# SamuelCancilla2/radar-point-cloud-tracking

Hardware: AMD Instinct MI355X
Metric: Mpoints/s clustered+tracked, 1024-echo synthetic frames; 1/2/4/8-GPU scaling (higher is better)
Workload: dtype u8 echo / f32 geometry / f64 distance

## Files before the change

### radar-point-cloud-tracking_amd/csrc/k1_emit.h

```cpp
#pragma once
#include <cstdint>

#if defined(__HIPCC__) || defined(__CUDACC__)
#define RPT_K1_HD __host__ __device__ __forceinline__
#else
#define RPT_K1_HD inline
#endif

namespace rpt {

constexpr int kStageSlots = 512;

struct EmitStride {
  uint32_t stride;
  uint32_t shift;
  bool pow2;
};
RPT_K1_HD EmitStride emit_stride(uint32_t stride) {
  return EmitStride{stride, (uint32_t)__builtin_ctz(stride), (stride & (stride - 1u)) == 0u};
}

struct EmitSpan {
  uint32_t first;
  uint32_t m;
  uint32_t rank0;
};

RPT_K1_HD uint32_t emit_ceil(uint32_t a, const EmitStride& es, uint32_t* rem) {
  const uint32_t q = es.pow2 ? (a >> es.shift) : a / es.stride;
  const uint32_t r = es.pow2 ? (a & (es.stride - 1u)) : a - q * es.stride;
  if (rem) *rem = r;
  return q + (r != 0u ? 1u : 0u);
}

RPT_K1_HD EmitSpan emit_span(uint32_t rank, uint32_t total, const EmitStride& es) {
  uint32_t rem;
  EmitSpan s;
  s.first = emit_ceil(rank, es, &rem);
  s.m = emit_ceil(rank + total, es, nullptr) - s.first;
  s.rank0 = rem != 0u ? es.stride - rem : 0u;
  return s;
}

RPT_K1_HD bool emit_staged(const EmitSpan& s) { return s.m != 0u && s.m <= (uint32_t)kStageSlots; }

}
```

### radar-point-cloud-tracking_amd/csrc/polar.hip

```cpp
#include <algorithm>
#include <cmath>
#include <cstdlib>

#include "common.h"
#include "k1_emit.h"

#pragma clang fp contract(off)

namespace rpt {
namespace {

constexpr int kBlock = 256;
constexpr int kWavesPerBlock = kBlock / kWave;

template <class T>
__device__ __forceinline__ float to_f(T v) {
  return (float)v;
}

template <class T>
struct Vec;
template <>
struct Vec<uint8_t> {
  static constexpr int N = 16;
// ... 275 lines not shown
    b.v[1] = max(b.v[1], part[4 * i + 1]);
    b.v[2] = min(b.v[2], part[4 * i + 2]);
    b.v[3] = max(b.v[3], part[4 * i + 3]);
  }
  __shared__ uint32_t sm[4 * kWavesPerBlock];
  b.store_block(out - 4 * blockIdx.x, sm, 1);
}

__device__ __forceinline__ void group_to_lds(GroupLds& L, int lane, const uint32_t (&m)[kGroupRows],
                                             const int (&incl)[kGroupRows],
                                             const uint4 (&vv)[kGroupRows]) {
#pragma unroll
  for (int k = 0; k < kGroupRows; ++k) {
    L.incl[k][lane] = (uint16_t)incl[k];
    L.mask[k][lane] = (uint16_t)m[k];
    *reinterpret_cast<uint4*>(&L.bytes[k][lane * 4]) = vv[k];
  }
  wave_lds_sync();
}

__device__ __forceinline__ uint32_t kept_entry(const GroupLds& L,
                                               const uint32_t (&rb)[kGroupRows + 1], uint32_t i) {
  const int k = (i >= rb[1]) + (i >= rb[2]) + (i >= rb[3]);
  const int ir = (int)(i - rb[k]);
  const uint16_t* inc = L.incl[k];
  int lo = 0;
#pragma unroll
  for (int step = 32; step > 0; step >>= 1)
    if (inc[lo + step - 1] <= ir) lo += step;
  const uint32_t msk = L.mask[k][lo];
  const int j = ir - ((int)inc[lo] - __popc(msk));
  const int bit = nth_bit16(msk, (uint32_t)j);
  const int bin = lo * 16 + bit;
  const uint32_t w = L.bytes[k][bin >> 2];
  return ((uint32_t)k << 18) | ((uint32_t)bin << 8) | __builtin_amdgcn_ubfe(w, 8u * (bin & 3), 8u);
}

__device__ __forceinline__ uint32_t phase_base(uint32_t ph, uint32_t total) {
  uint32_t b = 0u;
#pragma unroll
  for (uint32_t j = 0u; j < 3u; ++j) b += (j < ph) ? ((total + 3u - j) >> 2) : 0u;
  return b;
}
__device__ __forceinline__ uint32_t stage_pos(uint32_t i, uint32_t total, bool ph4) {
  return ph4 ? phase_base(i & 3u, total) + (i >> 2) : i;
}
struct StageBases {
  uint32_t b1, b2, b3;
  __device__ explicit StageBases(uint32_t total)
      : b1((total + 3u) >> 2), b2(b1 + ((total + 2u) >> 2)), b3(b2 + ((total + 1u) >> 2)) {}
  __device__ uint32_t pos(uint32_t i) const {
    const uint32_t r = i & 3u;
    return (r == 0u ? 0u : (r == 1u ? b1 : (r == 2u ? b2 : b3))) + (i >> 2);
  }
};

template <bool HI, bool STAGE>
__global__ __launch_bounds__(kBlock) void k_group_count_u8(const uint8_t* __restrict__ echo,
                                                          uint32_t n_groups, GroupMap gm,
                                                          uint32_t K,
                                                          int32_t* __restrict__ group_count,
                                                          uint32_t* __restrict__ entries,
                                                          int ph4) {
  const int lane = threadIdx.x & 63;
  const uint32_t wave0 = __builtin_amdgcn_readfirstlane(blockIdx.x * kWavesPerBlock +
                                                        threadIdx.x / 64);
  const uint32_t n_waves = gridDim.x * kWavesPerBlock;
  const uint32_t dq = n_waves / gm.gpf, dr = n_waves - dq * gm.gpf;
  uint32_t gf = wave0 / gm.gpf, gr = wave0 - gf * gm.gpf;
  for (uint32_t g0 = wave0; g0 < n_groups; g0 += n_waves) {
    const uint32_t grp = g0;
    const uint32_t f = gf;
    const int r0 = (int)gr * kGroupRows;
    const int64_t row0 = (int64_t)f * gm.rows + r0;
    const int nr = min(kGroupRows, gm.rows - r0);
    gf += dq;
    gr += dr;
    if (gr >= gm.gpf) {
      gr -= gm.gpf;
      ++gf;
    }
    uint4 v[kGroupRows];
#pragma unroll
    for (int k = 0; k < kGroupRows; ++k) {
      const u32x4 q = (k < nr) ? __builtin_nontemporal_load(reinterpret_cast<const u32x4*>(
                                     echo + (row0 + k) * 1024 + lane * 16))
                               : u32x4{0u, 0u, 0u, 0u};
      v[k] = make_uint4(q.x, q.y, q.z, q.w);
    }
    if constexpr (STAGE) {
      uint32_t m[kGroupRows];
      int incl[kGroupRows];
#pragma unroll
      for (int k = 0; k < kGroupRows; ++k)
        m[k] = (k < nr) ? mask16(keep_bits<HI>(v[k].x, K), keep_bits<HI>(v[k].y, K),
                                 keep_bits<HI>(v[k].z, K), keep_bits<HI>(v[k].w, K))
                        : 0u;
      static_assert(kGroupRows == 4, "rows are scanned in pairs");
      uint32_t rb[kGroupRows + 1];
      rb[0] = 0;
#pragma unroll
      for (int k = 0; k < kGroupRows; k += 2) {
        const int pair = wave_incl_scan_dpp(__popc(m[k]) | (__popc(m[k + 1]) << 16));
        incl[k] = pair & 0xffff;
        incl[k + 1] = (int)((uint32_t)pair >> 16);
        const uint32_t tot = (uint32_t)__builtin_amdgcn_readlane(pair, 63);
        rb[k + 1] = rb[k] + (tot & 0xffffu);
        rb[k + 2] = rb[k + 1] + (tot >> 16);
      }
      const uint32_t total = rb[kGroupRows];
      if (total != 0u && total <= (uint32_t)kStageSlots) {
        uint32_t* e = entries + (int64_t)grp * kStageSlots;
        __shared__ GroupLds s_lds[kWavesPerBlock];
        GroupLds& L = s_lds[threadIdx.x / 64];
        group_to_lds(L, lane, m, incl, v);
        const StageBases sb(total);
        for (uint32_t i = (uint32_t)lane; i < total; i += 64u)
          e[ph4 ? sb.pos(i) : i] = kept_entry(L, rb, i);
        wave_lds_sync();
      }
      if (lane == 0) group_count[grp] = (int32_t)total;
      continue;
    } else {
      uint32_t c = 0;
#pragma unroll
      for (int k = 0; k < kGroupRows; ++k) {
        if (k >= nr) break;
        c += __popc(keep_bits<HI>(v[k].x, K)) + __popc(keep_bits<HI>(v[k].y, K)) +
             __popc(keep_bits<HI>(v[k].z, K)) + __popc(keep_bits<HI>(v[k].w, K));
      }
      int s = (int)c;
#pragma unroll
      for (int off = 32; off > 0; off >>= 1) s += __shfl_xor(s, off);
      if (lane == 0) group_count[grp] = s;
    }
  }
}

template <int W>
struct CountTotals {
  uint32_t t[2][W];
};
template <bool HI, int W>
__global__ __launch_bounds__(64 * W) void k_group_count_u8_files(
    const uint8_t* __restrict__ echo, GroupMap gm, uint32_t K, EmitStride es,
    int32_t* __restrict__ group_count, uint32_t* __restrict__ entries) {
  __shared__ GroupLds s_lds[W];
  __shared__ CountTotals<W> s_tot;
  const int lane = threadIdx.x & 63;
  const uint32_t w = __builtin_amdgcn_readfirstlane(threadIdx.x / 64);
  const uint32_t f = blockIdx.x;
  const int64_t file_row0 = (int64_t)f * gm.rows;
  const uint32_t n_rounds = (gm.gpf + W - 1) / W;
  auto load_group = [&](uint32_t gi, u32x4 (&q)[kGroupRows]) -> int {
    const int r0 = (int)gi * kGroupRows;
    const int nr = gi < gm.gpf ? min(kGroupRows, gm.rows - r0) : 0;
#pragma unroll
    for (int k = 0; k < kGroupRows; ++k)
      q[k] = (k < nr) ? __builtin_nontemporal_load(reinterpret_cast<const u32x4*>(
                            echo + (file_row0 + r0 + k) * 1024 + lane * 16))
                      : u32x4{0u, 0u, 0u, 0u};
    return nr;
  };
  u32x4 nx[kGroupRows];
  int nr_next = load_group(w, nx);
  uint32_t rank = 0u;
  for (uint32_t r = 0u; r < n_rounds; ++r) {
    const uint32_t gi = r * W + w;
    const int nr = nr_next;
    uint4 v[kGroupRows];
#pragma unroll
    for (int k = 0; k < kGroupRows; ++k) v[k] = make_uint4(nx[k].x, nx[k].y, nx[k].z, nx[k].w);
    nr_next = load_group(gi + W, nx);
    uint32_t m[kGroupRows];
    int incl[kGroupRows];
#pragma unroll
    for (int k = 0; k < kGroupRows; ++k)
      m[k] = (k < nr) ? mask16(keep_bits<HI>(v[k].x, K), keep_bits<HI>(v[k].y, K),
                               keep_bits<HI>(v[k].z, K), keep_bits<HI>(v[k].w, K))
                      : 0u;
    static_assert(kGroupRows == 4, "rows are scanned in pairs");
    uint32_t rb[kGroupRows + 1];
    rb[0] = 0;
#pragma unroll
    for (int k = 0; k < kGroupRows; k += 2) {
      const int pair = wave_incl_scan_dpp(__popc(m[k]) | (__popc(m[k + 1]) << 16));
      incl[k] = pair & 0xffff;
      incl[k + 1] = (int)((uint32_t)pair >> 16);
      const uint32_t tot = (uint32_t)__builtin_amdgcn_readlane(pair, 63);
      rb[k + 1] = rb[k] + (tot & 0xffffu);
      rb[k + 2] = rb[k + 1] + (tot >> 16);
    }
    const uint32_t total = rb[kGroupRows];
    uint32_t my_rank = rank;
    if constexpr (W > 1) {
      const uint32_t par = r & 1u;
      if (lane == 0) s_tot.t[par][w] = total;
      __syncthreads();
      uint32_t below = 0u, all = 0u;
      static_assert(W <= 4, "the wave totals are summed as scalars");
#pragma unroll
      for (uint32_t j = 0u; j < (uint32_t)W; ++j) {
        const uint32_t t = __builtin_amdgcn_readfirstlane(s_tot.t[par][j]);
        below += j < w ? t : 0u;
        all += t;
      }
      my_rank += below;
      rank += all;
    } else {
      rank += total;
    }
    if (nr == 0) continue;
    const EmitSpan sp = emit_span(my_rank, total, es);
    const int64_t grp = (int64_t)f * gm.gpf + gi;
    if (emit_staged(sp)) {
      uint32_t* e = entries + grp * kStageSlots;
      GroupLds& L = s_lds[w];
      group_to_lds(L, lane, m, incl, v);
      for (uint32_t j = (uint32_t)lane; j < sp.m; j += 64u)
        e[j] = kept_entry(L, rb, sp.rank0 + j * es.stride);
      wave_lds_sync();
    }
    if (lane == 0) group_count[grp] = (int32_t)total;
  }
}

constexpr int64_t kCus = 256;
constexpr int64_t kEmittedMinFiles = 1500;
inline int64_t busiest_cu_files(int64_t n_files) { return (n_files + kCus - 1) / kCus; }
inline bool staged_emitted(int64_t n_files) {
  return n_files >= kEmittedMinFiles && n_files * 20 >= busiest_cu_files(n_files) * kCus * 19;
}

inline int count_waves_per_file(int64_t n_files) {
  const int64_t per_cu = busiest_cu_files(n_files);
  return per_cu <= 7 ? 4 : (per_cu <= 15 ? 2 : 1);
}

__global__ void k_file_counts_groups(const int64_t* __restrict__ gprefix, int64_t n_files,
                                     uint32_t gpf, int stride, int64_t* __restrict__ file_out) {
  for (int64_t f = (int64_t)blockIdx.x * blockDim.x + threadIdx.x; f < n_files;
       f += (int64_t)gridDim.x * blockDim.x) {
    const int64_t kept = gprefix[(f + 1) * gpf] - gprefix[f * gpf];
    file_out[f] = (kept + stride - 1) / stride;
  }
}

template <bool HI, bool STAGED, bool LIST = false, class VT = float>
__global__ __launch_bounds__(kBlock, 8) void k_group_write_u8(
    const uint8_t* __restrict__ echo, uint32_t n_groups, GroupMap gm, uint32_t K, int stride,
    const float* __restrict__ scale, const float* __restrict__ cos_t,
    const float* __restrict__ sin_t, const int32_t* __restrict__ gain,
    const int64_t* __restrict__ gprefix, const int64_t* __restrict__ file_offsets,
    int files_per_frame, float* __restrict__ x, float* __restrict__ y, VT* __restrict__ val,
    int32_t* __restrict__ gain_out, int32_t* __restrict__ pf_out, int64_t cap,
    const uint32_t* __restrict__ entries, bool emitted,
    const uint32_t* __restrict__ list = nullptr, const uint32_t* __restrict__ list_n = nullptr,
    uint32_t* __restrict__ bpart = nullptr) {
  __shared__ GroupLds s_lds[kWavesPerBlock];
  XyBounds xb;
  const int lane = threadIdx.x & 63;
  GroupLds& L = s_lds[threadIdx.x / 64];
  const uint32_t wave0 = blockIdx.x * kWavesPerBlock + threadIdx.x / 64;
  const uint32_t n_waves = gridDim.x * kWavesPerBlock;
  const uint32_t us = (uint32_t)stride;
  const EmitStride es = emit_stride(us);
  const float inv_bins = 1.0f / 1024.0f;
  const uint32_t n_items = LIST ? *list_n : n_groups;
  for (uint32_t g0 = wave0; g0 < n_items; g0 += n_waves) {
    const uint32_t grp = __builtin_amdgcn_readfirstlane(LIST ? list[g0] : g0);
    uint32_t f;
    int64_t row0;
    int nr;
    group_rows(gm, grp, &f, &row0, &nr);
    float g_sc = 0.f, g_c = 0.f, g_s = 0.f;
    if (lane < nr) {
      g_sc = scale[row0 + lane];
      g_c = cos_t[row0 + lane];
      g_s = sin_t[row0 + lane];
    }
    float r_sc[kGroupRows], r_c[kGroupRows], r_s[kGroupRows];
#pragma unroll
    for (int k = 0; k < kGroupRows; ++k) {
      r_sc[k] = __builtin_bit_cast(float, __builtin_amdgcn_readlane(__builtin_bit_cast(int, g_sc), k));
      r_c[k] = __builtin_bit_cast(float, __builtin_amdgcn_readlane(__builtin_bit_cast(int, g_c), k));
      r_s[k] = __builtin_bit_cast(float, __builtin_amdgcn_readlane(__builtin_bit_cast(int, g_s), k));
    }
    const int64_t gp0 = gprefix[grp];
    const uint32_t rank = (uint32_t)(gp0 - gprefix[(int64_t)f * gm.gpf]);
    const uint32_t total = (uint32_t)(gprefix[grp + 1] - gp0);
    const EmitSpan sp = emit_span(rank, total, es);
    if (sp.m == 0u) continue;
    const uint32_t first = sp.first, last = sp.first + sp.m;
    const int64_t out0 = file_offsets[f];
    const int32_t g = gain ? gain[f] : 0;
    const int32_t fr = (int32_t)(f / (uint32_t)files_per_frame);
    const bool staged =
        STAGED && (emitted ? emit_staged(sp) : total <= (uint32_t)kStageSlots);
    uint32_t rb[kGroupRows + 1];
    if (!staged) {
      uint4 vv[kGroupRows];
#pragma unroll
      for (int k = 0; k < kGroupRows; ++k)
        vv[k] = (k < nr) ? *reinterpret_cast<const uint4*>(echo + (row0 + k) * 1024 + lane * 16)
                         : make_uint4(0u, 0u, 0u, 0u);
      uint32_t m[kGroupRows];
      int incl[kGroupRows];
#pragma unroll
      for (int k = 0; k < kGroupRows; ++k) {
        m[k] = (k < nr) ? mask16(keep_bits<HI>(vv[k].x, K), keep_bits<HI>(vv[k].y, K),
                                 keep_bits<HI>(vv[k].z, K), keep_bits<HI>(vv[k].w, K))
                        : 0u;
        incl[k] = wave_incl_scan_dpp(__popc(m[k]));
      }
      rb[0] = 0;
#pragma unroll
      for (int k = 0; k < kGroupRows; ++k)
        rb[k + 1] = rb[k] + (uint32_t)__builtin_amdgcn_readlane(incl[k], 63);
      group_to_lds(L, lane, m, incl, vv);
    }
    const uint32_t* e = entries + (int64_t)grp * kStageSlots;
    for (uint32_t o = first + (uint32_t)lane; o < last; o += 64u) {
      const int64_t oo = out0 + o;
      if (oo >= cap) break;
      const uint32_t i = sp.rank0 + (o - first) * us;
      const uint32_t ent = !staged  ? kept_entry(L, rb, i)
                           : emitted ? e[o - first]
                                     : e[stage_pos(i, total, us == 4u)];
      const int rk = (int)(ent >> 18);
      const float sc = rk == 0 ? r_sc[0] : (rk == 1 ? r_sc[1] : (rk == 2 ? r_sc[2] : r_sc[3]));
      const float cc = rk == 0 ? r_c[0] : (rk == 1 ? r_c[1] : (rk == 2 ? r_c[2] : r_c[3]));
      const float ss = rk == 0 ? r_s[0] : (rk == 1 ? r_s[1] : (rk == 2 ? r_s[2] : r_s[3]));
      const float rr = sc * inv_bins * (float)((ent >> 8) & 1023u);
      const float px = rr * cc, py = rr * ss;
      x[oo] = px;
      y[oo] = py;
      if (bpart) xb.add(px, py);
      val[oo] = (VT)(ent & 0xffu);
      if (gain_out) gain_out[oo] = g;
      if (pf_out) pf_out[oo] = fr;
    }
    if (!staged) wave_lds_sync();
  }
  if (bpart)
    xb.store_block(bpart, reinterpret_cast<uint32_t*>(&s_lds[0]),
                   (int)(sizeof(GroupLds) / sizeof(uint32_t) / 4));
}

constexpr int kGsBits = 40;
constexpr uint64_t kGsMask = (1ull << kGsBits) - 1ull;
constexpr uint64_t kUnstaged = 1ull << 63;
constexpr int kTileOut = 1024;
constexpr int kOutPerThread = kTileOut / kBlock;
static_assert(kOutPerThread % 4 == 0, "k_expand_write stores a thread's outputs as 16-B vectors");
constexpr int kWin = 1024;

__global__ __launch_bounds__(kBlock) void k_group_starts(const int64_t* __restrict__ gprefix,
                                                        const int64_t* __restrict__ file_offsets,
                                                        uint32_t n_groups, uint32_t gpf,
                                                        uint32_t stride, bool emitted,
                                                        uint64_t* __restrict__ gword,
                                                        uint32_t* __restrict__ list,
                                                        uint32_t* __restrict__ list_n) {
  constexpr uint32_t kCap = 2048;
  __shared__ uint32_t s_list[kCap];
  __shared__ uint32_t s_n, s_base;
  if (threadIdx.x == 0) s_n = 0u;
  __syncthreads();
  const EmitStride es = emit_stride(stride);
  for (uint32_t b0 = blockIdx.x * kBlock; b0 < n_groups; b0 += gridDim.x * kBlock) {
    const uint32_t g = b0 + threadIdx.x;
    if (g < n_groups) {
      const uint32_t f = g / gpf;
      const int64_t p0 = gprefix[g];
      const uint32_t rank = (uint32_t)(p0 - gprefix[(int64_t)f * gpf]);
      const uint32_t total = (uint32_t)(gprefix[g + 1] - p0);
      const EmitSpan sp = emit_span(rank, total, es);
      const uint64_t gs = (uint64_t)file_offsets[f] + sp.first;
      const uint64_t phase = emitted       ? 0ull
                             : stride == 4u ? (uint64_t)phase_base(sp.rank0, total)
                                            : (uint64_t)sp.rank0;
      const bool un =
          sp.m != 0u && !(emitted ? emit_staged(sp) : total <= (uint32_t)kStageSlots);
      gword[g] = gs | (phase << kGsBits) | (un ? kUnstaged : 0ull);
      if (un) {
        const uint32_t slot = atomicAdd(&s_n, 1u);
        if (slot < kCap)
          s_list[slot] = g;
        else
          list[atomicAdd(list_n, 1u)] = g;
      }
    }
  }
  __syncthreads();
  const uint32_t m = min(s_n, kCap);
  if (threadIdx.x == 0 && m) s_base = atomicAdd(list_n, m);
  __syncthreads();
  for (uint32_t i = threadIdx.x; i < m; i += kBlock) list[s_base + i] = s_list[i];
}

__device__ uint32_t wave_find_group(const uint64_t* __restrict__ gword, uint32_t lo, uint32_t hi,
                                    uint64_t O) {
  const uint32_t lane = threadIdx.x & 63u;
  while (hi - lo > 1u) {
    const uint32_t step = (hi - lo + 63u) / 64u;
    const uint32_t idx = lo + lane * step;
    const bool le = idx < hi && (gword[idx] & kGsMask) <= O;
    const uint64_t m = __ballot(le);
    const uint32_t top = 63u - (uint32_t)__clzll((long long)m);
    lo = __builtin_amdgcn_readfirstlane(lo + top * step);
    hi = min(hi, lo + step);
  }
  return lo;
}

__device__ uint32_t thread_find_group(const uint64_t* __restrict__ gword, uint32_t lo,
                                      uint32_t hi, uint64_t O) {
  while (hi - lo > 1u) {
    const uint32_t mid = lo + (hi - lo) / 2u;
    if ((gword[mid] & kGsMask) <= O)
      lo = mid;
    else
      hi = mid;
  }
  return lo;
}

__device__ __forceinline__ uint32_t lds_find(const uint64_t* s_win, uint32_t wn, uint64_t O) {
  uint32_t lo = 0u;
#pragma unroll
  for (uint32_t step = kWin / 2; step > 0u; step >>= 1)
    if (lo + step < wn && (s_win[lo + step] & kGsMask) <= O) lo += step;
  return lo;
}

template <bool VEC, class VT = float>
__global__ __launch_bounds__(kBlock) void k_expand_write(
    const uint64_t* __restrict__ gword, uint32_t n_groups, GroupMap gm, uint32_t estep,
    const float* __restrict__ scale, const float* __restrict__ cos_t,
    const float* __restrict__ sin_t, const int32_t* __restrict__ gain,
    const int64_t* __restrict__ total_out, int files_per_frame, float* __restrict__ x,
    float* __restrict__ y, VT* __restrict__ val, int32_t* __restrict__ gain_out,
    int32_t* __restrict__ pf_out, int64_t cap, const uint32_t* __restrict__ entries,
    uint32_t* __restrict__ bpart = nullptr) {
  __shared__ uint64_t s_win[kWin];
  __shared__ uint32_t s_glo;
  const int64_t total = min(*total_out, cap);
  const int64_t n_tiles = (total + kTileOut - 1) / kTileOut;
  const int64_t t0 = n_tiles * blockIdx.x / gridDim.x;
  const int64_t t1 = n_tiles * (blockIdx.x + 1) / gridDim.x;
  if (t0 >= t1) {
    if (bpart && threadIdx.x < 4)
      bpart[4 * blockIdx.x + threadIdx.x] = (threadIdx.x & 1) ? 0u : 0xffffffffu;
    return;
  }
  if (threadIdx.x < 64) {
    const uint32_t g = wave_find_group(gword, 0u, n_groups, (uint64_t)t0 * kTileOut);
    if (threadIdx.x == 0) s_glo = g;
  }
  __syncthreads();
  constexpr int kWinPer = kWin / kBlock;
  uint64_t wv[kWinPer];
  auto load_win = [&](uint32_t glo_) {
    const uint32_t wn_ = min((uint32_t)kWin, n_groups - glo_);
#pragma unroll
    for (int q = 0; q < kWinPer; ++q) {
      const uint32_t j = threadIdx.x + q * kBlock;
      wv[q] = j < wn_ ? gword[glo_ + j] : ~0ull;
    }
  };
  auto store_win = [&]() {
#pragma unroll
    for (int q = 0; q < kWinPer; ++q) s_win[threadIdx.x + q * kBlock] = wv[q];
  };
  uint32_t glo = s_glo;
  XyBounds xb;
  load_win(glo);
  store_win();
  __syncthreads();
  const float inv_bins = 1.0f / 1024.0f;
  for (int64_t t = t0; t < t1; ++t) {
    const uint32_t wn = min((uint32_t)kWin, n_groups - glo);
    const bool truncated = glo + wn < n_groups;
    const uint64_t O0 = (uint64_t)t * kTileOut;
    auto word = [&](uint32_t g) -> uint64_t {
      return (g - glo < wn) ? s_win[g - glo] : gword[g];
    };
    auto next_gs = [&](uint32_t g) -> uint64_t {
      return g + 1u < n_groups ? (word(g + 1u) & kGsMask) : ~0ull;
    };
    const uint64_t Ob = O0 + (uint64_t)threadIdx.x * kOutPerThread;
    uint32_t grp[kOutPerThread], idx[kOutPerThread];
    bool ok[kOutPerThread];
    if ((int64_t)Ob < total) {
      const uint32_t j = lds_find(s_win, wn, Ob);
      uint32_t g = (j == wn - 1u && truncated) ? thread_find_group(gword, glo + j, n_groups, Ob)
                                               : glo + j;
      uint64_t w = word(g), nx = next_gs(g);
#pragma unroll
      for (int k = 0; k < kOutPerThread; ++k) {
        const uint64_t O = Ob + k;
        const bool in = (int64_t)O < total;
        while (in && O >= nx) {
          ++g;
          w = word(g);
          nx = next_gs(g);
        }
        ok[k] = in && !(w & kUnstaged);
        grp[k] = g;
        const uint32_t d = (uint32_t)O - (uint32_t)w;
        idx[k] = d * estep + (uint32_t)((w & ~kUnstaged) >> kGsBits);
      }
    } else {
#pragma unroll
      for (int k = 0; k < kOutPerThread; ++k) {
        ok[k] = false;
        grp[k] = glo;
        idx[k] = 0u;
      }
    }
    if (threadIdx.x == 0 && t + 1 < t1) {
      const uint64_t On = O0 + kTileOut;
      const uint32_t j = lds_find(s_win, wn, On);
      s_glo = (j == wn - 1u && truncated) ? thread_find_group(gword, glo + j, n_groups, On)
                                          : glo + j;
    }
    __syncthreads();
    if (t + 1 < t1) {
      glo = s_glo;
      load_win(glo);
    }
    uint32_t ent[kOutPerThread];
#pragma unroll
    for (int k = 0; k < kOutPerThread; ++k) {
      const uint32_t e = entries[ok[k] ? (int64_t)grp[k] * kStageSlots + idx[k] : 0];
      ent[k] = ok[k] ? e : 0u;
    }
    float sc[kOutPerThread], cc[kOutPerThread], ss[kOutPerThread];
    uint32_t fl[kOutPerThread], pfl[kOutPerThread];
    const uint32_t f0 = grp[0] / gm.gpf, r0 = grp[0] - f0 * gm.gpf;
    const uint32_t fpf = (uint32_t)files_per_frame, p0 = f0 / fpf, q0 = f0 - p0 * fpf;
#pragma unroll
    for (int k = 0; k < kOutPerThread; ++k) {
      uint32_t f = f0, r = r0 + (grp[k] - grp[0]);
      while (r >= gm.gpf) {
        r -= gm.gpf;
        ++f;
      }
      uint32_t pf = p0, q = q0 + (f - f0);
      while (q >= fpf) {
        q -= fpf;
        ++pf;
      }
      fl[k] = f;
      pfl[k] = pf;
      const int64_t row = (int64_t)f * gm.rows + (int64_t)r * kGroupRows + (ent[k] >> 18);
      sc[k] = scale[row];
      cc[k] = cos_t[row];
      ss[k] = sin_t[row];
    }
    float ox[kOutPerThread], oy[kOutPerThread], ov[kOutPerThread];
    int32_t og[kOutPerThread], op[kOutPerThread];
    bool all_ok = true;
#pragma unroll
    for (int k = 0; k < kOutPerThread; ++k) {
      const float rr = sc[k] * inv_bins * (float)((ent[k] >> 8) & 1023u);
      ox[k] = rr * cc[k];
      oy[k] = rr * ss[k];
      ov[k] = (float)(ent[k] & 0xffu);
      og[k] = gain ? gain[fl[k]] : 0;
      op[k] = (int32_t)pfl[k];
      all_ok = all_ok && ok[k];
      if (bpart && ok[k]) xb.add(ox[k], oy[k]);
    }
    if (VEC && all_ok) {
#pragma unroll
      for (int h = 0; h < kOutPerThread; h += 4) {
        const uint64_t o = Ob + h;
        *reinterpret_cast<float4*>(x + o) = make_float4(ox[h], ox[h + 1], ox[h + 2], ox[h + 3]);
        *reinterpret_cast<float4*>(y + o) = make_float4(oy[h], oy[h + 1], oy[h + 2], oy[h + 3]);
        if constexpr (sizeof(VT) == 1)
          *reinterpret_cast<uint32_t*>(val + o) =
              (ent[h] & 0xffu) | ((ent[h + 1] & 0xffu) << 8) | ((ent[h + 2] & 0xffu) << 16) |
              ((ent[h + 3] & 0xffu) << 24);
        else
          *reinterpret_cast<float4*>(val + o) = make_float4(ov[h], ov[h + 1], ov[h + 2], ov[h + 3]);
        if (gain_out)
          *reinterpret_cast<int4*>(gain_out + o) = make_int4(og[h], og[h + 1], og[h + 2], og[h + 3]);
        if (pf_out)
          *reinterpret_cast<int4*>(pf_out + o) = make_int4(op[h], op[h + 1], op[h + 2], op[h + 3]);
      }
    } else {
#pragma unroll
      for (int k = 0; k < kOutPerThread; ++k) {
        if (!ok[k]) continue;
        const uint64_t oo = Ob + k;
        x[oo] = ox[k];
        y[oo] = oy[k];
        val[oo] = (VT)(ent[k] & 0xffu);
        if (gain_out) gain_out[oo] = og[k];
        if (pf_out) pf_out[oo] = op[k];
      }
    }
    if (t + 1 < t1) store_win();
    __syncthreads();
  }
  if (bpart) xb.store_block(bpart, reinterpret_cast<uint32_t*>(s_win), 1);
}

inline int u8_threshold(float thr) {
  if (!(thr == thr)) return 255;
  const double f = std::floor((double)thr);
  return f < -1.0 ? -1 : (f > 255.0 ? 255 : (int)f);
}

template <class T>
constexpr bool is_u8() { return false; }
template <>
constexpr bool is_u8<uint8_t>() { return true; }

template <class T>
bool grouped_u8(const T* echo, int bins) {
  return is_u8<T>() && bins == 1024 && (uintptr_t)echo % 16 == 0;
}

inline uint32_t u8_k(int T) {
  return (uint32_t)(T <= 127 ? 127 - T : 255 - T) * 0x01010101u;
}

constexpr int kExpandBlocks = 2048;
constexpr int kListBlocks = 2048;

template <class T>
int32_t count_impl(const T* echo, int64_t n_files, int rows, int bins, float thr, int stride,
                   int64_t* row_prefix, int64_t* file_offsets, int64_t* total_host,
                   hipStream_t st, uint32_t* entries = nullptr) {
  const int64_t n_rows = n_files * rows;
  if ((int64_t)rows * bins >= (int64_t(1) << 32) || n_rows >= (int64_t(1) << 32)) {
    set_error("rpt_polar_count: rows*bins and n_files*rows must be < 2^32");
    return RPT_ENOTSUP;
  }
  const bool grouped = grouped_u8(echo, bins);
  const GroupMap gm{(uint32_t)((rows + kGroupRows - 1) / kGroupRows), rows};
  const int64_t n_units = grouped ? n_files * (int64_t)gm.gpf : n_rows;
  Scratch& sc = scratch(st);
  Budget b;
  b.add<int32_t>(n_units);
  b.add<int64_t>(n_files);
  RPT_TRY(sc.reserve(b.bytes, st));
  int32_t* rc = sc.carve_n<int32_t>(n_units);
  int64_t* fo = sc.carve_n<int64_t>(n_files);
  const bool vec = (bins % (64 * Vec<T>::N) == 0) && ((uintptr_t)echo % 16 == 0);
  const int grid = grid_for(n_units, kWavesPerBlock, 16384);
  if (grouped) {
    const int T8 = u8_threshold(thr);
    const auto* e8 = reinterpret_cast<const uint8_t*>(echo);
#define RPT_K1C(HI, S)                                                                    \
  hipLaunchKernelGGL((k_group_count_u8<HI, S>), dim3(grid), dim3(kBlock), 0, st, e8,        \
                     (uint32_t)n_units, gm, u8_k(T8), rc, entries, stride == 4 ? 1 : 0)
#define RPT_K1F(HI, W)                                                                    \
  hipLaunchKernelGGL((k_group_count_u8_files<HI, W>), dim3((unsigned)n_files), dim3(64 * W), 0, \
                     st, e8, gm, u8_k(T8), emit_stride((uint32_t)stride), rc, entries)
#define RPT_K1FW(W)       \
  if (T8 <= 127)          \
    RPT_K1F(false, W);    \
  else                    \
    RPT_K1F(true, W)
    if (entries && staged_emitted(n_files)) {
      switch (count_waves_per_file(n_files)) {
        case 4: RPT_K1FW(4); break;
        case 2: RPT_K1FW(2); break;
        default: RPT_K1FW(1); break;
      }
    } else if (entries) {
      if (T8 <= 127)
        RPT_K1C(false, true);
      else
        RPT_K1C(true, true);
    } else if (T8 <= 127) {
      RPT_K1C(false, false);
    } else {
      RPT_K1C(true, false);
    }
#undef RPT_K1FW
#undef RPT_K1F
#undef RPT_K1C
  } else if (vec) {
    hipLaunchKernelGGL((k_row_count<T, true>), dim3(grid), dim3(kBlock), 0, st, echo, n_rows,
                       bins, thr, rc);
  } else {
    hipLaunchKernelGGL((k_row_count<T, false>), dim3(grid), dim3(kBlock), 0, st, echo, n_rows,
                       bins, thr, rc);
  }
  RPT_CHECK_LAUNCH();
  RPT_TRY(exclusive_scan_total_i32_to_i64(rc, row_prefix, n_units, st));
  if (grouped)
    hipLaunchKernelGGL(k_file_counts_groups, dim3(grid_for(n_files, 256, 1024)), dim3(256), 0, st,
                       row_prefix, n_files, gm.gpf, stride, fo);
  else
    hipLaunchKernelGGL(k_file_counts, dim3(grid_for(n_files, 256, 1024)), dim3(256), 0, st,
                       row_prefix, n_files, rows, stride, fo);
  RPT_CHECK_LAUNCH();
  RPT_TRY(exclusive_scan_total_i64(fo, file_offsets, n_files, st));
  if (total_host) {
    RPT_HIP(hipMemcpyAsync(total_host, file_offsets + n_files, sizeof(int64_t),
                           hipMemcpyDeviceToHost, st));
    RPT_TRY(wait_stream(st));
  }
  return RPT_OK;
}

template <class T, class VT = float>
int32_t write_impl(const T* echo, int64_t n_files, int rows, int bins, float thr, int stride,
                   RowGeo geo, const int32_t* gain, const int64_t* row_prefix,
                   const int64_t* file_offsets, int fpf, float* x, float* y, VT* v,
                   int32_t* gout, int32_t* pf, hipStream_t st, int64_t cap = INT64_MAX,
                   const uint32_t* entries = nullptr, uint32_t* bnd = nullptr,
                   bool* bnd_done = nullptr) {
  if (bnd_done) *bnd_done = false;
  const int64_t n_rows = n_files * rows;
  if ((int64_t)rows * bins >= (int64_t(1) << 32) || n_rows >= (int64_t(1) << 32) || stride < 1 ||
      fpf < 1) {
    set_error("rpt_polar_write: rows*bins and n_files*rows must be < 2^32, stride/fpf >= 1");
    return RPT_ENOTSUP;
  }
  const bool vec = (bins % (64 * Vec<T>::N) == 0) && ((uintptr_t)echo % 16 == 0);
  if (grouped_u8(echo, bins) && geo.scale) {
    const GroupMap gm{(uint32_t)((rows + kGroupRows - 1) / kGroupRows), rows};
    const int64_t n_groups = n_files * (int64_t)gm.gpf;
    const int grid = grid_for(n_groups, kWavesPerBlock, 16384);
    const int T8 = u8_threshold(thr);
    const auto* e8 = reinterpret_cast<const uint8_t*>(echo);
    const bool emitted = staged_emitted(n_files);
    if (entries && ab().k1_expand && stride < (1 << 23) &&
        n_files * (int64_t)rows * 1024 < (int64_t(1) << kGsBits)) {
      Scratch& sc = scratch(st);
      Budget b;
      b.add<uint64_t>(n_groups);
      b.add<uint32_t>(n_groups);
      RPT_TRY(sc.reserve(b.bytes, st));
      uint64_t* gword = sc.carve_n<uint64_t>(n_groups);
      uint32_t* list = sc.carve_n<uint32_t>(n_groups);
      uint32_t* list_n = nullptr;
      RPT_TRY(zero_n(st, 1, &list_n));
      hipLaunchKernelGGL(k_group_starts, dim3(grid_for(n_groups, kBlock, 4096)), dim3(kBlock), 0,
                         st, row_prefix, file_offsets, (uint32_t)n_groups, gm.gpf,
                         (uint32_t)stride, emitted, gword, list, list_n);
      RPT_CHECK_LAUNCH();
      auto al16 = [](const void* q) { return ((uintptr_t)q & 15u) == 0; };
      const bool vec4 = al16(x) && al16(y) && al16(v) && (!gout || al16(gout)) && (!pf || al16(pf));
      const uint32_t estep = (emitted || stride == 4) ? 1u : (uint32_t)stride;
      if (vec4)
        hipLaunchKernelGGL((k_expand_write<true, VT>), dim3(kExpandBlocks), dim3(kBlock), 0, st, gword,
                           (uint32_t)n_groups, gm, estep, geo.scale, geo.cos_t, geo.sin_t, gain,
                           file_offsets + n_files, fpf, x, y, v, gout, pf, cap, entries,
                           bnd ? bnd + 4 : nullptr);
      else
        hipLaunchKernelGGL((k_expand_write<false, VT>), dim3(kExpandBlocks), dim3(kBlock), 0, st,
                           gword, (uint32_t)n_groups, gm, estep, geo.scale, geo.cos_t, geo.sin_t,
                           gain, file_offsets + n_files, fpf, x, y, v, gout, pf, cap, entries,
                           bnd ? bnd + 4 : nullptr);
      RPT_CHECK_LAUNCH();
      const int lgrid = std::min(grid, kListBlocks);
#define RPT_K1L(HI)                                                                            \
  hipLaunchKernelGGL((k_group_write_u8<HI, false, true, VT>), dim3(lgrid), dim3(kBlock), 0, st, e8, \
                     (uint32_t)n_groups, gm, u8_k(T8), stride, geo.scale, geo.cos_t, geo.sin_t,  \
                     gain, row_prefix, file_offsets, fpf, x, y, v, gout, pf, cap, entries,       \
                     emitted, list, list_n, bnd ? bnd + 4 + 4 * kExpandBlocks : nullptr)
      if (T8 <= 127)
        RPT_K1L(false);
      else
        RPT_K1L(true);
#undef RPT_K1L
      if (bnd) {
        hipLaunchKernelGGL(k_bounds_parts, dim3(1), dim3(kBlock), 0, st, bnd + 4,
                           kExpandBlocks + lgrid, bnd);
        if (bnd_done) *bnd_done = true;
      }
      RPT_CHECK_LAUNCH();
      return RPT_OK;
    }
#define RPT_K1W(HI, M)                                                                       \
  hipLaunchKernelGGL((k_group_write_u8<HI, M, false, VT>), dim3(grid), dim3(kBlock), 0, st, e8,          \
                     (uint32_t)n_groups, gm, u8_k(T8), stride, geo.scale, geo.cos_t, geo.sin_t, \
                     gain, row_prefix, file_offsets, fpf, x, y, v, gout, pf, cap, entries, emitted)
    if (entries) {
      if (T8 <= 127)
        RPT_K1W(false, true);
      else
        RPT_K1W(true, true);
    } else if (T8 <= 127) {
      RPT_K1W(false, false);
    } else {
      RPT_K1W(true, false);
    }
#undef RPT_K1W
  } else if (cap != INT64_MAX) {
    set_error("rpt_polar_write: a capacity-bounded write needs u8 sweeps of 1024 bins");
    return RPT_ENOTSUP;
  } else if (grouped_u8(echo, bins)) {
    set_error("rpt_polar_write: u8 sweeps take per-row scale geometry");
    return RPT_ENOTSUP;
  } else if constexpr (sizeof(VT) == 1) {
    set_error("rpt_polar_write: u8 intensities need u8 sweeps of 1024 bins");
    return RPT_ENOTSUP;
  } else if (vec) {
    const int grid = grid_for(n_rows, kWavesPerBlock, 16384);
    hipLaunchKernelGGL((k_row_write<T, true>), dim3(grid), dim3(kBlock), 0, st, echo, n_rows,
                       rows, bins, thr, stride, geo, gain, row_prefix, file_offsets, fpf, x, y,
                       v, gout, pf);
  } else {
    const int grid = grid_for(n_rows, kWavesPerBlock, 16384);
    hipLaunchKernelGGL((k_row_write<T, false>), dim3(grid), dim3(kBlock), 0, st, echo, n_rows,
                       rows, bins, thr, stride, geo, gain, row_prefix, file_offsets, fpf, x, y,
                       v, gout, pf);
  }
  RPT_CHECK_LAUNCH();
  return RPT_OK;
}

__global__ void k_frame_times(const int32_t* __restrict__ pf, int64_t n,
                              const int64_t* __restrict__ ids, float* __restrict__ t,
                              const int64_t* __restrict__ n_dev) {
  if (n_dev) n = *n_dev;
  for (int64_t i = (int64_t)blockIdx.x * blockDim.x + threadIdx.x; i < n;
       i += (int64_t)gridDim.x * blockDim.x) {
    const int32_t f = pf[i];
    t[i] = (float)(ids ? ids[f] : (int64_t)f);
  }
}

__global__ void k_frame_fill(const int64_t* __restrict__ off, float* __restrict__ t,
                             int32_t* __restrict__ pf) {
  const int32_t f = blockIdx.x;
  const int64_t hi = off[f + 1];
  for (int64_t i = off[f] + threadIdx.x; i < hi; i += blockDim.x) {
    if (t) t[i] = (float)f;
    if (pf) pf[i] = f;
  }
}

__global__ void k_bytes_to_float(const uint8_t* __restrict__ in, int64_t n,
                                 float* __restrict__ out) {
  for (int64_t i = (int64_t)blockIdx.x * blockDim.x + threadIdx.x; i < n;
       i += (int64_t)gridDim.x * blockDim.x)
    out[i] = (float)in[i];
}

__global__ void k_polar_dense(const float* __restrict__ cos_t, const float* __restrict__ sin_t,
                              const float* __restrict__ ranges, int64_t rows, int64_t bins,
                              float* __restrict__ x, float* __restrict__ y) {
  const int64_t n = rows * bins;
  for (int64_t i = (int64_t)blockIdx.x * blockDim.x + threadIdx.x; i < n;
       i += (int64_t)gridDim.x * blockDim.x) {
    const int64_t r = i / bins;
    const float rr = ranges[i];
    x[i] = rr * cos_t[r];
    y[i] = rr * sin_t[r];
  }
}

__global__ void k_colors(const uint8_t* __restrict__ colors, int64_t n,
                         const float* __restrict__ pal, int n_pal, float* __restrict__ out) {
  for (int64_t i = (int64_t)blockIdx.x * blockDim.x + threadIdx.x; i < n;
       i += (int64_t)gridDim.x * blockDim.x) {
    const float r = colors[3 * i], g = colors[3 * i + 1], b = colors[3 * i + 2];
    int best = 0;
    float bd = 0.f;
    for (int k = 0; k < n_pal; ++k) {
      const float d0 = r - pal[3 * k], d1 = g - pal[3 * k + 1], d2 = b - pal[3 * k + 2];
      float d = d0 * d0;
      d = d + d1 * d1;
      d = d + d2 * d2;
      if (k == 0 || d < bd) {
        bd = d;
        best = k;
      }
    }
    out[i] = (float)best;
  }
}

__device__ __forceinline__ uint64_t splitmix64(uint64_t z) {
  z += 0x9E3779B97F4A7C15ull;
  z = (z ^ (z >> 30)) * 0xBF58476D1CE4E5B9ull;
  z = (z ^ (z >> 27)) * 0x94D049BB133111EBull;
  return z ^ (z >> 31);
}

constexpr int kMaxTargets = 256;

__global__ __launch_bounds__(kBlock) void k_synth(rpt_synth_params p, int64_t frame0,
                                                 int64_t n_frames, const float* __restrict__ cos_t,
                                                 const float* __restrict__ sin_t,
                                                 const uint32_t* __restrict__ clutter_thresh,
                                                 const float* __restrict__ targets,
                                                 const int32_t* __restrict__ trows,
                                                 const int32_t* __restrict__ tbins,
                                                 uint8_t* __restrict__ echo) {
  __shared__ int hits[kMaxTargets];
  __shared__ int n_hits;
  const int64_t n_rows_total = n_frames * p.n_gains * p.rows;
  for (int64_t rr = blockIdx.x; rr < n_rows_total; rr += gridDim.x) {
    const int row = (int)(rr % p.rows);
    const int64_t fg = rr / p.rows;
    const int gi = (int)(fg % p.n_gains);
    const int64_t fl = fg / p.n_gains;
    const int64_t fa = frame0 + fl;
    __syncthreads();
    if (threadIdx.x == 0) n_hits = 0;
    __syncthreads();
    for (int k = threadIdx.x; k < p.n_targets; k += blockDim.x) {
      const int32_t* tr = trows + (fl * p.n_targets + k) * 2;
      if (row >= tr[0] && row <= tr[1]) hits[atomicAdd(&n_hits, 1)] = k;
// ... 269 lines not shown
```

Baseline: 8833.

## Stage emitted entries contiguously per file and expand with file-level stream kernel

Staged entries move from per-group slots to one contiguous per-file buffer indexed by output position. Each entry now carries its absolute row bits, so a new streaming expand kernel can find the owning file by binary search and read entries linearly. Per-group start words are replaced by a per-file staged cutoff. This aims to cut per-group bookkeeping and get coalesced reads in the expand pass, at the cost of extra file searches and a new limit on row count (at most 16384 rows).

```diff
diff --git a/radar-point-cloud-tracking_amd/csrc/k1_emit.h b/radar-point-cloud-tracking_amd/csrc/k1_emit.h
--- a/radar-point-cloud-tracking_amd/csrc/k1_emit.h
+++ b/radar-point-cloud-tracking_amd/csrc/k1_emit.h
@@ -44,4 +44,24 @@
 
 RPT_K1_HD bool emit_staged(const EmitSpan& s) { return s.m != 0u && s.m <= (uint32_t)kStageSlots; }
 
+RPT_K1_HD bool emit_staged_file(const EmitSpan& s, uint32_t cap) {
+  return s.m != 0u && s.first + s.m <= cap;
 }
+RPT_K1_HD bool emit_unstaged_file(const EmitSpan& s, uint32_t cap) {
+  return s.m != 0u && s.first + s.m > cap;
+}
+RPT_K1_HD uint32_t emit_staged_out(uint32_t so, const EmitSpan& s, uint32_t cap) {
+  return (emit_unstaged_file(s, cap) && s.first < so) ? s.first : so;
+}
+
+constexpr int64_t kCus = 256;
+constexpr int64_t kEmittedMinFiles = 1500;
+constexpr int kEntryRowBits = 14;
+constexpr int kEmittedMaxRows = 1 << kEntryRowBits;
+inline int64_t busiest_cu_files(int64_t n_files) { return (n_files + kCus - 1) / kCus; }
+inline bool staged_emitted(int64_t n_files, int64_t rows) {
+  return n_files >= kEmittedMinFiles && n_files * 20 >= busiest_cu_files(n_files) * kCus * 19 &&
+         rows <= kEmittedMaxRows;
+}
+
+}
diff --git a/radar-point-cloud-tracking_amd/csrc/polar.hip b/radar-point-cloud-tracking_amd/csrc/polar.hip
--- a/radar-point-cloud-tracking_amd/csrc/polar.hip
+++ b/radar-point-cloud-tracking_amd/csrc/polar.hip
@@ -451,6 +451,7 @@
   const uint32_t f = blockIdx.x;
   const int64_t file_row0 = (int64_t)f * gm.rows;
   const uint32_t n_rounds = (gm.gpf + W - 1) / W;
+  const uint32_t fcap = gm.gpf * (uint32_t)kStageSlots;
   auto load_group = [&](uint32_t gi, u32x4 (&q)[kGroupRows]) -> int {
     const int r0 = (int)gi * kGroupRows;
     const int nr = gi < gm.gpf ? min(kGroupRows, gm.rows - r0) : 0;
@@ -512,24 +513,19 @@
     if (nr == 0) continue;
     const EmitSpan sp = emit_span(my_rank, total, es);
     const int64_t grp = (int64_t)f * gm.gpf + gi;
-    if (emit_staged(sp)) {
-      uint32_t* e = entries + grp * kStageSlots;
+    if (emit_staged_file(sp, fcap)) {
+      uint32_t* e = entries + (int64_t)f * fcap + sp.first;
+      const uint32_t row_bits = (gi * kGroupRows) << 18;
       GroupLds& L = s_lds[w];
       group_to_lds(L, lane, m, incl, v);
       for (uint32_t j = (uint32_t)lane; j < sp.m; j += 64u)
-        e[j] = kept_entry(L, rb, sp.rank0 + j * es.stride);
+        e[j] = kept_entry(L, rb, sp.rank0 + j * es.stride) | row_bits;
       wave_lds_sync();
     }
     if (lane == 0) group_count[grp] = (int32_t)total;
   }
 }
 
-constexpr int64_t kCus = 256;
-constexpr int64_t kEmittedMinFiles = 1500;
-inline int64_t busiest_cu_files(int64_t n_files) { return (n_files + kCus - 1) / kCus; }
-inline bool staged_emitted(int64_t n_files) {
-  return n_files >= kEmittedMinFiles && n_files * 20 >= busiest_cu_files(n_files) * kCus * 19;
-}
 
 inline int count_waves_per_file(int64_t n_files) {
   const int64_t per_cu = busiest_cu_files(n_files);
@@ -594,8 +590,9 @@
     const int64_t out0 = file_offsets[f];
     const int32_t g = gain ? gain[f] : 0;
     const int32_t fr = (int32_t)(f / (uint32_t)files_per_frame);
-    const bool staged =
-        STAGED && (emitted ? emit_staged(sp) : total <= (uint32_t)kStageSlots);
+    const uint32_t fcap = gm.gpf * (uint32_t)kStageSlots;
+    const bool staged = STAGED && (emitted ? emit_staged_file(sp, fcap)
+                                           : total <= (uint32_t)kStageSlots);
     uint32_t rb[kGroupRows + 1];
     if (!staged) {
       uint4 vv[kGroupRows];
@@ -618,7 +615,8 @@
         rb[k + 1] = rb[k] + (uint32_t)__builtin_amdgcn_readlane(incl[k], 63);
       group_to_lds(L, lane, m, incl, vv);
     }
-    const uint32_t* e = entries + (int64_t)grp * kStageSlots;
+    const uint32_t* e = entries + ((STAGED && emitted) ? (int64_t)f * fcap + first
+                                                       : (int64_t)grp * kStageSlots);
     for (uint32_t o = first + (uint32_t)lane; o < last; o += 64u) {
       const int64_t oo = out0 + o;
       if (oo >= cap) break;
@@ -626,7 +624,7 @@
       const uint32_t ent = !staged  ? kept_entry(L, rb, i)
                            : emitted ? e[o - first]
                                      : e[stage_pos(i, total, us == 4u)];
-      const int rk = (int)(ent >> 18);
+      const int rk = (int)((ent >> 18) & 3u);
       const float sc = rk == 0 ? r_sc[0] : (rk == 1 ? r_sc[1] : (rk == 2 ? r_sc[2] : r_sc[3]));
       const float cc = rk == 0 ? r_c[0] : (rk == 1 ? r_c[1] : (rk == 2 ? r_c[2] : r_c[3]));
       const float ss = rk == 0 ? r_s[0] : (rk == 1 ? r_s[1] : (rk == 2 ? r_s[2] : r_s[3]));
@@ -657,7 +655,7 @@
 __global__ __launch_bounds__(kBlock) void k_group_starts(const int64_t* __restrict__ gprefix,
                                                         const int64_t* __restrict__ file_offsets,
                                                         uint32_t n_groups, uint32_t gpf,
-                                                        uint32_t stride, bool emitted,
+                                                        uint32_t stride,
                                                         uint64_t* __restrict__ gword,
                                                         uint32_t* __restrict__ list,
                                                         uint32_t* __restrict__ list_n) {
@@ -676,11 +674,9 @@
       const uint32_t total = (uint32_t)(gprefix[g + 1] - p0);
       const EmitSpan sp = emit_span(rank, total, es);
       const uint64_t gs = (uint64_t)file_offsets[f] + sp.first;
-      const uint64_t phase = emitted       ? 0ull
-                             : stride == 4u ? (uint64_t)phase_base(sp.rank0, total)
-                                            : (uint64_t)sp.rank0;
-      const bool un =
-          sp.m != 0u && !(emitted ? emit_staged(sp) : total <= (uint32_t)kStageSlots);
+      const uint64_t phase = stride == 4u ? (uint64_t)phase_base(sp.rank0, total)
+                                          : (uint64_t)sp.rank0;
+      const bool un = sp.m != 0u && total > (uint32_t)kStageSlots;
       gword[g] = gs | (phase << kGsBits) | (un ? kUnstaged : 0ull);
       if (un) {
         const uint32_t slot = atomicAdd(&s_n, 1u);
@@ -907,6 +903,263 @@
   if (bpart) xb.store_block(bpart, reinterpret_cast<uint32_t*>(s_win), 1);
 }
 
+__global__ __launch_bounds__(kBlock) void k_file_staged(const int64_t* __restrict__ gprefix,
+                                                       const int64_t* __restrict__ file_offsets,
+                                                       uint32_t n_files, uint32_t gpf,
+                                                       uint32_t stride,
+                                                       uint32_t* __restrict__ staged_out,
+                                                       uint32_t* __restrict__ list,
+                                                       uint32_t* __restrict__ list_n) {
+  const uint32_t lane = threadIdx.x & 63u;
+  const uint32_t fcap = gpf * (uint32_t)kStageSlots;
+  for (uint32_t f = __builtin_amdgcn_readfirstlane(blockIdx.x * kWavesPerBlock + threadIdx.x / 64);
+       f < n_files; f += gridDim.x * kWavesPerBlock) {
+    const uint32_t count = (uint32_t)(file_offsets[f + 1] - file_offsets[f]);
+    uint32_t so = count;
+    if (count > fcap) {
+      const EmitStride es = emit_stride(stride);
+      const int64_t* gp = gprefix + (int64_t)f * gpf;
+      const int64_t p00 = gp[0];
+      auto unstaged = [&](uint32_t g, EmitSpan* sp) -> bool {
+        if (g >= gpf) return false;
+        const int64_t p0 = gp[g];
+        *sp = emit_span((uint32_t)(p0 - p00), (uint32_t)(gp[g + 1] - p0), es);
+        return emit_unstaged_file(*sp, fcap);
+      };
+      uint32_t n_un = 0u;
+      for (uint32_t g0 = 0u; g0 < gpf; g0 += 64u) {
+        EmitSpan sp{};
+        if (unstaged(g0 + lane, &sp)) {
+          so = emit_staged_out(so, sp, fcap);
+          ++n_un;
+        }
+      }
+#pragma unroll
+      for (int off = 32; off > 0; off >>= 1) {
+        so = min(so, (uint32_t)__shfl_xor((int)so, off));
+        n_un += (uint32_t)__shfl_xor((int)n_un, off);
+      }
+      uint32_t base = 0u;
+      if (lane == 0u) base = atomicAdd(list_n, n_un);
+      base = __builtin_amdgcn_readfirstlane(base);
+      for (uint32_t g0 = 0u; g0 < gpf; g0 += 64u) {
+        EmitSpan sp{};
+        const bool un = unstaged(g0 + lane, &sp);
+        const uint64_t b = __ballot(un);
+        if (un) list[base + (uint32_t)rank_in_mask(b)] = f * gpf + g0 + lane;
+        base += (uint32_t)__popcll(b);
+      }
+    }
+    if (lane == 0u) staged_out[f] = so;
+  }
+}
+
+constexpr int kFWin = kBlock;
+
+__device__ uint32_t wave_find_file(const int64_t* __restrict__ fo, uint32_t lo, uint32_t hi,
+                                   int64_t O) {
+  const uint32_t lane = threadIdx.x & 63u;
+  while (hi - lo > 1u) {
+    const uint32_t step = (hi - lo + 63u) / 64u;
+    const uint32_t idx = lo + lane * step;
+    const bool le = idx < hi && fo[idx] <= O;
+    const uint64_t m = __ballot(le);
+    const uint32_t top = 63u - (uint32_t)__clzll((long long)m);
+    lo = __builtin_amdgcn_readfirstlane(lo + top * step);
+    hi = min(hi, lo + step);
+  }
+  return lo;
+}
+
+__device__ uint32_t thread_find_file(const int64_t* __restrict__ fo, uint32_t lo, uint32_t hi,
+                                     int64_t O) {
+  while (hi - lo > 1u) {
+    const uint32_t mid = lo + (hi - lo) / 2u;
+    if (fo[mid] <= O)
+      lo = mid;
+    else
+      hi = mid;
+  }
+  return lo;
+}
+
+__device__ __forceinline__ uint32_t lds_find_file(const int64_t* s_fo, uint32_t wn, int64_t O) {
+  uint32_t lo = 0u;
+#pragma unroll
+  for (uint32_t step = kFWin / 2; step > 0u; step >>= 1)
+    if (lo + step < wn && s_fo[lo + step] <= O) lo += step;
+  return lo;
+}
+
+template <bool VEC, class VT = float>
+__global__ __launch_bounds__(kBlock) void k_expand_stream(
+    const int64_t* __restrict__ file_offsets, uint32_t n_files,
+    const uint32_t* __restrict__ staged_out, GroupMap gm, const float* __restrict__ scale,
+    const float* __restrict__ cos_t, const float* __restrict__ sin_t,
+    const int32_t* __restrict__ gain, int files_per_frame, float* __restrict__ x,
+    float* __restrict__ y, VT* __restrict__ val, int32_t* __restrict__ gain_out,
+    int32_t* __restrict__ pf_out, int64_t cap, const uint32_t* __restrict__ entries,
+    uint32_t* __restrict__ bpart = nullptr) {
+  __shared__ int64_t s_fo[kFWin];
+  __shared__ uint32_t s_flo;
+  const uint32_t n_off = n_files + 1u;
+  const int64_t total = min(file_offsets[n_files], cap);
+  const int64_t n_tiles = (total + kTileOut - 1) / kTileOut;
+  const int64_t t0 = n_tiles * blockIdx.x / gridDim.x;
+  const int64_t t1 = n_tiles * (blockIdx.x + 1) / gridDim.x;
+  if (t0 >= t1) {
+    if (bpart && threadIdx.x < 4)
+      bpart[4 * blockIdx.x + threadIdx.x] = (threadIdx.x & 1) ? 0u : 0xffffffffu;
+    return;
+  }
+  if (threadIdx.x < 64) {
+    const uint32_t f = wave_find_file(file_offsets, 0u, n_off, t0 * kTileOut);
+    if (threadIdx.x == 0) s_flo = f;
+  }
+  __syncthreads();
+  int64_t wv;
+  auto load_win = [&](uint32_t flo_) {
+    wv = threadIdx.x < min((uint32_t)kFWin, n_off - flo_) ? file_offsets[flo_ + threadIdx.x]
+                                                          : INT64_MAX;
+  };
+  uint32_t flo = s_flo;
+  XyBounds xb;
+  load_win(flo);
+  s_fo[threadIdx.x] = wv;
+  __syncthreads();
+  const uint32_t fcap = gm.gpf * (uint32_t)kStageSlots;
+  const uint32_t fpf = (uint32_t)files_per_frame;
+  const float inv_bins = 1.0f / 1024.0f;
+  for (int64_t t = t0; t < t1; ++t) {
+    const uint32_t wn = min((uint32_t)kFWin, n_off - flo);
+    const bool truncated = flo + wn < n_off;
+    const int64_t O0 = t * kTileOut;
+    auto off = [&](uint32_t i) -> int64_t {
+      return (i - flo < wn) ? s_fo[i - flo] : file_offsets[i];
+    };
+    const int64_t Ob = O0 + (int64_t)threadIdx.x * kOutPerThread;
+    uint32_t fl[kOutPerThread], oi[kOutPerThread];
+    bool in[kOutPerThread];
+    if (Ob < total) {
+      const uint32_t j = lds_find_file(s_fo, wn, Ob);
+      uint32_t f = (j == wn - 1u && truncated) ? thread_find_file(file_offsets, flo + j, n_off, Ob)
+                                               : flo + j;
+      int64_t base = off(f), nx = off(f + 1u);
+#pragma unroll
+      for (int k = 0; k < kOutPerThread; ++k) {
+        const int64_t O = Ob + k;
+        in[k] = O < total;
+        while (in[k] && O >= nx) {
+          ++f;
+          base = nx;
+          nx = off(f + 1u);
+        }
+        fl[k] = f;
+        oi[k] = (uint32_t)(O - base);
+      }
+    } else {
+#pragma unroll
+      for (int k = 0; k < kOutPerThread; ++k) {
+        in[k] = false;
+        fl[k] = flo;
+        oi[k] = 0u;
+      }
+    }
+    if (threadIdx.x == 0 && t + 1 < t1) {
+      const int64_t On = O0 + kTileOut;
+      const uint32_t j = lds_find_file(s_fo, wn, On);
+      s_flo = (j == wn - 1u && truncated) ? thread_find_file(file_offsets, flo + j, n_off, On)
+                                          : flo + j;
+    }
+    __syncthreads();
+    if (t + 1 < t1) {
+      flo = s_flo;
+      load_win(flo);
+    }
+    uint32_t ent[kOutPerThread];
+    bool ok[kOutPerThread];
+#pragma unroll
+    for (int k = 0; k < kOutPerThread; ++k) {
+      const uint32_t so = staged_out[fl[k]];
+      const uint32_t e =
+          entries[(in[k] && oi[k] < fcap) ? (int64_t)fl[k] * fcap + oi[k] : (int64_t)0];
+      ok[k] = in[k] && oi[k] < so;
+      ent[k] = ok[k] ? e : 0u;
+    }
+    float sc[kOutPerThread], cc[kOutPerThread], ss[kOutPerThread];
+    uint32_t pfl[kOutPerThread];
+    uint32_t pf = fl[0] / fpf, q = fl[0] - pf * fpf;
+#pragma unroll
+    for (int k = 0; k < kOutPerThread; ++k) {
+      if (k > 0) {
+        q += fl[k] - fl[k - 1];
+        if (q >= fpf) {
+          if (q < 2u * fpf) {
+            q -= fpf;
+            ++pf;
+          } else {
+            const uint32_t d = q / fpf;
+            pf += d;
+            q -= d * fpf;
+          }
+        }
+      }
+      pfl[k] = pf;
+      const int64_t row = (int64_t)fl[k] * gm.rows + (ent[k] >> 18);
+      sc[k] = scale[row];
+      cc[k] = cos_t[row];
+      ss[k] = sin_t[row];
+    }
+    float ox[kOutPerThread], oy[kOutPerThread];
+    int32_t og[kOutPerThread], op[kOutPerThread];
+    bool all_ok = true;
+#pragma unroll
+    for (int k = 0; k < kOutPerThread; ++k) {
+      const float rr = sc[k] * inv_bins * (float)((ent[k] >> 8) & 1023u);
+      ox[k] = rr * cc[k];
+      oy[k] = rr * ss[k];
+      og[k] = gain ? gain[fl[k]] : 0;
+      op[k] = (int32_t)pfl[k];
+      all_ok = all_ok && ok[k];
+      if (bpart && ok[k]) xb.add(ox[k], oy[k]);
+    }
+    if (VEC && all_ok) {
+#pragma unroll
+      for (int h = 0; h < kOutPerThread; h += 4) {
+        const int64_t o = Ob + h;
+        *reinterpret_cast<float4*>(x + o) = make_float4(ox[h], ox[h + 1], ox[h + 2], ox[h + 3]);
+        *reinterpret_cast<float4*>(y + o) = make_float4(oy[h], oy[h + 1], oy[h + 2], oy[h + 3]);
+        if constexpr (sizeof(VT) == 1)
+          *reinterpret_cast<uint32_t*>(val + o) =
+              (ent[h] & 0xffu) | ((ent[h + 1] & 0xffu) << 8) | ((ent[h + 2] & 0xffu) << 16) |
+              ((ent[h + 3] & 0xffu) << 24);
+        else
+          *reinterpret_cast<float4*>(val + o) =
+              make_float4((float)(ent[h] & 0xffu), (float)(ent[h + 1] & 0xffu),
+                          (float)(ent[h + 2] & 0xffu), (float)(ent[h + 3] & 0xffu));
+        if (gain_out)
+          *reinterpret_cast<int4*>(gain_out + o) = make_int4(og[h], og[h + 1], og[h + 2], og[h + 3]);
+        if (pf_out)
+          *reinterpret_cast<int4*>(pf_out + o) = make_int4(op[h], op[h + 1], op[h + 2], op[h + 3]);
+      }
+    } else {
+#pragma unroll
+      for (int k = 0; k < kOutPerThread; ++k) {
+        if (!ok[k]) continue;
+        const int64_t oo = Ob + k;
+        x[oo] = ox[k];
+        y[oo] = oy[k];
+        val[oo] = (VT)(ent[k] & 0xffu);
+        if (gain_out) gain_out[oo] = og[k];
+        if (pf_out) pf_out[oo] = op[k];
+      }
+    }
+    if (t + 1 < t1) s_fo[threadIdx.x] = wv;
+    __syncthreads();
+  }
+  if (bpart) xb.store_block(bpart, reinterpret_cast<uint32_t*>(s_fo), 1);
+}
+
 inline int u8_threshold(float thr) {
   if (!(thr == thr)) return 255;
   const double f = std::floor((double)thr);
@@ -965,7 +1218,7 @@
     RPT_K1F(false, W);    \
   else                    \
     RPT_K1F(true, W)
-    if (entries && staged_emitted(n_files)) {
+    if (entries && staged_emitted(n_files, rows)) {
       switch (count_waves_per_file(n_files)) {
         case 4: RPT_K1FW(4); break;
         case 2: RPT_K1FW(2); break;
@@ -1030,35 +1283,56 @@
     const int grid = grid_for(n_groups, kWavesPerBlock, 16384);
     const int T8 = u8_threshold(thr);
     const auto* e8 = reinterpret_cast<const uint8_t*>(echo);
-    const bool emitted = staged_emitted(n_files);
-    if (entries && ab().k1_expand && stride < (1 << 23) &&
-        n_files * (int64_t)rows * 1024 < (int64_t(1) << kGsBits)) {
+    const bool emitted = staged_emitted(n_files, rows);
+    if (entries && ab().k1_expand &&
+        (emitted || (stride < (1 << 23) &&
+                     n_files * (int64_t)rows * 1024 < (int64_t(1) << kGsBits)))) {
       Scratch& sc = scratch(st);
       Budget b;
-      b.add<uint64_t>(n_groups);
+      if (emitted)
+        b.add<uint32_t>(n_files);
+      else
+        b.add<uint64_t>(n_groups);
       b.add<uint32_t>(n_groups);
       RPT_TRY(sc.reserve(b.bytes, st));
-      uint64_t* gword = sc.carve_n<uint64_t>(n_groups);
+      uint64_t* gword = emitted ? nullptr : sc.carve_n<uint64_t>(n_groups);
+      uint32_t* staged_out = emitted ? sc.carve_n<uint32_t>(n_files) : nullptr;
       uint32_t* list = sc.carve_n<uint32_t>(n_groups);
       uint32_t* list_n = nullptr;
       RPT_TRY(zero_n(st, 1, &list_n));
-      hipLaunchKernelGGL(k_group_starts, dim3(grid_for(n_groups, kBlock, 4096)), dim3(kBlock), 0,
-                         st, row_prefix, file_offsets, (uint32_t)n_groups, gm.gpf,
-                         (uint32_t)stride, emitted, gword, list, list_n);
+      if (emitted)
+        hipLaunchKernelGGL(k_file_staged, dim3(grid_for(n_files, kWavesPerBlock)), dim3(kBlock), 0,
+                           st, row_prefix, file_offsets, (uint32_t)n_files, gm.gpf,
+                           (uint32_t)stride, staged_out, list, list_n);
+      else
+        hipLaunchKernelGGL(k_group_starts, dim3(grid_for(n_groups, kBlock, 4096)), dim3(kBlock), 0,
+                           st, row_prefix, file_offsets, (uint32_t)n_groups, gm.gpf,
+                           (uint32_t)stride, gword, list, list_n);
       RPT_CHECK_LAUNCH();
       auto al16 = [](const void* q) { return ((uintptr_t)q & 15u) == 0; };
       const bool vec4 = al16(x) && al16(y) && al16(v) && (!gout || al16(gout)) && (!pf || al16(pf));
-      const uint32_t estep = (emitted || stride == 4) ? 1u : (uint32_t)stride;
-      if (vec4)
-        hipLaunchKernelGGL((k_expand_write<true, VT>), dim3(kExpandBlocks), dim3(kBlock), 0, st, gword,
-                           (uint32_t)n_groups, gm, estep, geo.scale, geo.cos_t, geo.sin_t, gain,
-                           file_offsets + n_files, fpf, x, y, v, gout, pf, cap, entries,
-                           bnd ? bnd + 4 : nullptr);
-      else
-        hipLaunchKernelGGL((k_expand_write<false, VT>), dim3(kExpandBlocks), dim3(kBlock), 0, st,
-                           gword, (uint32_t)n_groups, gm, estep, geo.scale, geo.cos_t, geo.sin_t,
-                           gain, file_offsets + n_files, fpf, x, y, v, gout, pf, cap, entries,
-                           bnd ? bnd + 4 : nullptr);
+      const uint32_t estep = stride == 4 ? 1u : (uint32_t)stride;
+      uint32_t* bpart = bnd ? bnd + 4 : nullptr;
+#define RPT_K1S(VEC)                                                                             \
+  hipLaunchKernelGGL((k_expand_stream<VEC, VT>), dim3(kExpandBlocks), dim3(kBlock), 0, st,        \
+                     file_offsets, (uint32_t)n_files, staged_out, gm, geo.scale, geo.cos_t,      \
+                     geo.sin_t, gain, fpf, x, y, v, gout, pf, cap, entries, bpart)
+#define RPT_K1E(VEC)                                                                             \
+  hipLaunchKernelGGL((k_expand_write<VEC, VT>), dim3(kExpandBlocks), dim3(kBlock), 0, st, gword,  \
+                     (uint32_t)n_groups, gm, estep, geo.scale, geo.cos_t, geo.sin_t, gain,       \
+                     file_offsets + n_files, fpf, x, y, v, gout, pf, cap, entries, bpart)
+      if (emitted) {
+        if (vec4)
+          RPT_K1S(true);
+        else
+          RPT_K1S(false);
+      } else if (vec4) {
+        RPT_K1E(true);
+      } else {
+        RPT_K1E(false);
+      }
+#undef RPT_K1E
+#undef RPT_K1S
       RPT_CHECK_LAUNCH();
       const int lgrid = std::min(grid, kListBlocks);
 #define RPT_K1L(HI)                                                                            \
```

Measured after the change: 9040, median of 6. +2.3%, better.
